# fractalclockwork/CS267_HW3

Hardware: NVIDIA B200
Metric: kmers_per_s_insert_plus_traverse (higher is better)
Workload: dtype u128

## Files before the change

### cs267_hw3_b200/csrc/capi.cu

```cuda
#include <algorithm>
#include <cmath>
#include <cstdio>
#include <cstdlib>
#include <cstring>
#include <string>
#include <vector>

#include <cub/device/device_radix_sort.cuh>

#include "../../include/kh_capi.h"
#include "kernels.cuh"
#include "ctable.cuh"

using namespace kh;

namespace {

struct DevBuf {
    void* p = nullptr;
    size_t cap = 0;
};

enum { EV_INS0, EV_INS1, EV_AS0, EV_WALK, EV_RANK, EV_AS1, EV_PACK0, EV_PACK1, EV_CLR0, EV_CLR1, EV_STAGE1, EV_BUILD0, EV_BUILD1, EV_COUNT };

// ... 33 lines not shown
    kh_stats stats = {};
    std::string err;
    int sm_count = 148, walk_blocks_per_sm = 0, rank_blocks_per_sm = 0;
    u64 last_contig_bytes = 0, last_n_contigs = 0;
    struct CtState {
        bool on = false, sealed = false, sharded = false, attr_set = false, connected = false;
        bool assembled = false;
        CtGeom g = {};
        CtCaps caps = {};
        CtPeers pe = {};
        u32 epoch = 0;
        u64 n_local_max = 0, n_total = 0, n_starts_max = 0, out_cap = 0;
        u64 n_starts_host = 0;
        DevBuf xin_vals, xin_chunk, xin_cnt, xin_done, xout_cursor, extra_vals, extra_chunk, extra_cnt, fine, chunk_cursor,
               chunk_base, pool_off, seg_base, ext_key, meta, pool, inbox, inbox_cnt, out_cursor, flags,
               answers, req_seg, g_link, g_meta, g_pool, g_hdr;
        bool slow = false;
        void* ipc_opened[kMaxRanks][24] = {};
    } ct;
    int ct_env = 1;
};

namespace {

int fail(kh_table* t, int status, const std::string& msg) {
    if (t) t->err = msg;
    return status;
}

#define KH_CUDA(t, expr)                                                                         \
    do {                                                                                         \
// ... 440 lines not shown
    KH_TRY(ensure(t, c.chunk_base, (C + 2) * sizeof(u32)));
    KH_TRY(ensure(t, c.pool_off, (C + 2) * sizeof(u32)));
    KH_TRY(ensure(t, c.seg_base, (C + 1) * sizeof(u32)));
    KH_TRY(ensure(t, c.pool, c.caps.pool_cap + 64));
    KH_TRY(ensure(t, c.inbox, (u64)world * c.caps.inbox_cap * sizeof(CtReq<W>)));
    KH_TRY(ensure(t, c.inbox_cnt, kMaxRanks * sizeof(u32)));
    KH_TRY(ensure(t, c.out_cursor, kMaxRanks * sizeof(u32)));
    KH_TRY(ensure(t, c.flags, 2 * kMaxRanks * sizeof(u32)));
    c.caps.g_seg_stride = world > 1 ? ((n_local_max + 1 + n_exp + 64 + 15) & ~15ull) : 0;
    c.caps.g_pool_stride = world > 1 ? ((c.caps.pool_cap + 64 + 15) & ~15ull) : 0;
    KH_TRY(ensure(t, c.answers, std::max<u64>(16, (u64)(world > 1 ? world : 0) * c.caps.inbox_cap * sizeof(u32))));
    KH_TRY(ensure(t, c.req_seg, std::max<u64>(16, (u64)(world > 1 ? world : 0) * c.caps.inbox_cap * sizeof(u32))));
    KH_TRY(ensure(t, c.g_link, std::max<u64>(16, (u64)world * c.caps.g_seg_stride * sizeof(u64))));
    KH_TRY(ensure(t, c.g_meta, std::max<u64>(16, (u64)world * c.caps.g_seg_stride * sizeof(u64))));
    KH_TRY(ensure(t, c.g_pool, std::max<u64>(16, (u64)world * c.caps.g_pool_stride)));
    KH_TRY(ensure(t, c.g_hdr, 2 * kMaxRanks * sizeof(u32)));
    if (sharded) {
        KH_TRY(ensure(t, t->link, seg_cap * sizeof(u64)));
        KH_TRY(ensure(t, c.meta, seg_cap * sizeof(u64)));
        KH_TRY(ensure(t, c.ext_key, seg_cap * sizeof(V)));
        KH_TRY(ensure(t, t->contig_len, (hcap + 2) * sizeof(u32)));
        KH_TRY(ensure(t, t->contig_pre, (hcap + 2) * sizeof(u32)));
        KH_TRY(ensure(t, t->contig_off, (hcap + 2) * sizeof(u64)));
        KH_TRY(ensure(t, t->out, c.out_cap));
        KH_TRY(ensure(t, t->starts, (hcap + 1) * sizeof(V)));
        const u64 ntiles = (n_local_max + kInsTile - 1) / kInsTile + 1;
        KH_TRY(ensure(t, t->mask, (ntiles + 1) * (kInsTile / 32) * sizeof(u32)));
        KH_TRY(ensure(t, t->tile_counts, (ntiles + 1) * sizeof(u32)));
        KH_TRY(ensure(t, t->tile_offs, (ntiles + 1) * sizeof(u64)));
        KH_TRY(ensure(t, t->scan_blocks, ((std::max(ntiles, hcap + 2) + kScanTile - 1) / kScanTile + 2) * sizeof(u64)));
    }
    KH_TRY(ct_reset_staging(t));
    KH_CUDA(t, cudaMemsetAsync(c.inbox_cnt.p, 0, kMaxRanks * sizeof(u32), t->stream));
    KH_CUDA(t, cudaMemsetAsync(c.flags.p, 0, 2 * kMaxRanks * sizeof(u32), t->stream));
// ... 83 lines not shown
    }
    return ct_barrier(t);
}
template <int W>
int ct_seal_build(kh_table* t) {
    typedef typename Slot<W>::value_t V;
    auto& c = t->ct;
    const u32 C = c.g.chunks_per_rank;
    if (!c.sharded) {
        const u64 hcap = c.n_starts_host + 1;
        const u64 seg_cap = hcap + std::max<u64>(t->n_expected, 1) + 64;
        if (seg_cap >= 0xFFFFFF00ull) return fail(t, KH_ERR_ARG, "too many segments for 32-bit ids");
        c.caps.hcap = (u32)hcap; c.caps.seg_cap = (u32)seg_cap;
        KH_TRY(ensure(t, t->link, seg_cap * sizeof(u64)));
        KH_TRY(ensure(t, c.meta, seg_cap * sizeof(u64)));
        KH_TRY(ensure(t, c.ext_key, seg_cap * sizeof(V)));
        ct_set_self(t);
    }
    ct_init_seal_kernel<<<1, 1, 0, t->stream>>>(t->d_ctr, c.caps.hcap);
    if (c.pe.world > 1) {
        u32* done = static_cast<u32*>(c.xin_done.p);
        ct_xin_scatter_kernel<W><<<(unsigned)t->sm_count * 8, 256, 0, t->stream>>>(
            static_cast<const V*>(c.xin_vals.p), static_cast<const u32*>(c.xin_chunk.p), static_cast<const u32*>(c.xin_cnt.p), done,
            c.g, c.caps, static_cast<u32*>(c.chunk_cursor.p), static_cast<V*>(c.fine.p), t->d_ctr);
        ct_extra_kernel<W><<<64, 256, 0, t->stream>>>(static_cast<const V*>(c.extra_vals.p), static_cast<const u32*>(c.extra_chunk.p),
                                                      static_cast<const u32*>(c.extra_cnt.p), done + kMaxRanks, c.caps, C,
                                                      static_cast<u32*>(c.chunk_cursor.p), static_cast<V*>(c.fine.p), t->d_ctr);
        ct_mark_filed_kernel<<<1, 32, 0, t->stream>>>(static_cast<const u32*>(c.xin_cnt.p), done, static_cast<const u32*>(c.extra_cnt.p),
                                                      done + kMaxRanks, c.caps, c.pe.world);
        t->n_launches += 3;
    }
    ct_layout_kernel<<<1, 1024, 0, t->stream>>>(static_cast<const u32*>(c.chunk_cursor.p), C, c.g, c.caps, (u32)Slot<W>::kPerBucket,
                                                CtBuild<W>::kMaxSlots, static_cast<u32*>(c.chunk_base.p), static_cast<u32*>(c.pool_off.p), t->d_ctr);
    t->n_launches += 2;
    KH_CUDA(t, cudaEventRecord(t->ev[EV_BUILD0], t->stream));
    ct_build_kernel<W><<<C, kCtBuildThreads, CtBuild<W>::kSmem, t->stream>>>(
        static_cast<const V*>(c.fine.p), static_cast<const u32*>(c.chunk_cursor.p), static_cast<const u32*>(c.chunk_base.p),
        static_cast<const u32*>(c.pool_off.p), static_cast<V*>(t->table), static_cast<u32*>(c.seg_base.p),
        static_cast<u64*>(t->link.p), static_cast<u64*>(c.meta.p), static_cast<V*>(c.ext_key.p),
        static_cast<unsigned char*>(c.pool.p), c.g, c.caps, t->d_ctr);
    KH_CUDA(t, cudaGetLastError());
    KH_CUDA(t, cudaEventRecord(t->ev[EV_BUILD1], t->stream));
    t->have_build = true;
    c.sealed = true;
    return KH_OK;
}

constexpr int kCtMaxRounds = 24;
constexpr int kCtParts = 8 + kCtMaxRounds;
constexpr u32 kCtWalkMaxSteps = 512;

template <int W>
int ct_assemble_part(kh_table* t, int part) {
    typedef typename Slot<W>::value_t V;
    auto& c = t->ct;
    const unsigned gb = (unsigned)t->sm_count * 8;
    u64* link = static_cast<u64*>(t->link.p);
    CtGathered gt = {};
    for (int r = 0; r < c.pe.world; ++r) {
        const bool me = r == c.pe.rank;
        gt.link[r] = me ? link : static_cast<const u64*>(c.g_link.p) + (u64)r * c.caps.g_seg_stride;
        gt.meta[r] = me ? static_cast<const u64*>(c.meta.p) : static_cast<const u64*>(c.g_meta.p) + (u64)r * c.caps.g_seg_stride;
        gt.pool[r] = me ? static_cast<const unsigned char*>(c.pool.p) : static_cast<const unsigned char*>(c.g_pool.p) + (u64)r * c.caps.g_pool_stride;
    }
    switch (part) {
    case 0:
        if (c.assembled) { c.sealed = false; c.assembled = false; }
        c.slow = false;
        KH_CUDA(t, cudaEventRecord(t->ev[EV_AS0], t->stream));
        if (!c.sealed) return ct_seal_publish<W>(t);
        return ct_barrier(t);
    case 1: {
        if (!c.sealed) { KH_TRY(ct_seal_build<W>(t)); KH_CUDA(t, cudaEventRecord(t->ev[EV_INS1], t->stream)); t->have_ins = true; }
        if (!c.sharded) {
            const u64 hc = c.n_starts_host;
            KH_TRY(ensure(t, t->contig_len, (hc + 3) * sizeof(u32)));
            KH_TRY(ensure(t, t->contig_pre, (hc + 3) * sizeof(u32)));
            KH_TRY(ensure(t, t->contig_off, (hc + 3) * sizeof(u64)));
// ... 30 lines not shown
        }
        return ct_barrier(t);
    case 3:
        if (c.pe.world > 1) {
            ct_apply_kernel<<<gb, 256, 0, t->stream>>>(link, static_cast<const u32*>(c.answers.p), static_cast<const u32*>(c.req_seg.p),
                                                       static_cast<const u32*>(c.out_cursor.p), c.caps, c.pe.world, c.pe.rank);
            ct_gather_kernel<<<gb, 256, 0, t->stream>>>(c.pe, c.caps, link, static_cast<const u64*>(c.meta.p), static_cast<const unsigned char*>(c.pool.p),
                                                        static_cast<const u32*>(c.pool_off.p), c.g.chunks_per_rank, t->d_ctr, 1);
            KH_CUDA(t, cudaStreamWaitEvent(t->stream, t->ev_gathered, 0));
            KH_CUDA(t, cudaGetLastError());
            t->n_launches += 2;
        }
        KH_CUDA(t, cudaEventRecord(t->ev[EV_WALK], t->stream));
        return ct_barrier(t);
    case 4:
        ct_walk_len_kernel<<<gb, 256, 0, t->stream>>>(gt, link, c.caps, t->k, kCtWalkMaxSteps, static_cast<u32*>(t->contig_len.p), t->d_ctr);
        KH_CUDA(t, cudaGetLastError());
        ++t->n_launches;
        return ct_barrier(t, -2);
    case 5: {
        KH_TRY(device_scan(t, static_cast<u32*>(t->contig_len.p), (u64)c.caps.hcap + 1, static_cast<u64*>(t->contig_off.p), &t->d_ctr->contig_bytes));
        KH_CUDA(t, cudaEventRecord(t->ev[EV_RANK], t->stream));
        ct_walk_emit_kernel<W><<<gb, 256, 0, t->stream>>>(gt, link, static_cast<const V*>(t->starts.p), c.caps, t->k, static_cast<const u32*>(t->contig_len.p),
                                                          static_cast<const u64*>(t->contig_off.p), c.out_cap, static_cast<char*>(t->out.p), t->d_ctr);
        KH_CUDA(t, cudaGetLastError());
        ++t->n_launches;
        KH_CUDA(t, cudaEventRecord(t->ev[EV_AS1], t->stream));
        t->have_as = true;
        return KH_OK;
    }
    case 6: {
        KH_TRY(read_counters(t));
        c.slow = (c.pe.world > 1 ? t->h_ctr->use_jump : t->h_ctr->need_jump) != 0;
        if (!c.slow) return KH_OK;
        c.assembled = true;
        ct_rank_round_kernel<<<gb, 256, 0, t->stream>>>(c.pe, link, c.caps, t->d_ctr, t->d_ctr->flags, 0);
        KH_CUDA(t, cudaGetLastError());
        ++t->n_launches;
        return ct_barrier(t, 0);
    }
    case 6 + kCtMaxRounds: {
        if (!c.slow) return KH_OK;
        ct_reset_nodes_kernel<<<1, 1, 0, t->stream>>>(t->d_ctr);
        ct_lengths_kernel<<<gb, 256, 0, t->stream>>>(c.pe, link, c.caps, t->k, static_cast<u32*>(t->contig_len.p),
                                                     static_cast<u32*>(t->contig_pre.p), t->d_ctr);
        ct_claim_kernel<<<gb, 256, 0, t->stream>>>(c.pe, link, c.caps, static_cast<const u32*>(t->contig_len.p), t->d_ctr);
        KH_CUDA(t, cudaGetLastError());
        t->n_launches += 3;
        KH_TRY(device_scan(t, static_cast<u32*>(t->contig_len.p), (u64)c.caps.hcap + 1, static_cast<u64*>(t->contig_off.p), &t->d_ctr->contig_bytes));
        KH_CUDA(t, cudaEventRecord(t->ev[EV_RANK], t->stream));
        return ct_barrier(t);
    }
    case 7 + kCtMaxRounds:
        if (!c.slow) return KH_OK;
        ct_emit_kernel<<<gb, 256, 0, t->stream>>>(c.pe, link, static_cast<const u64*>(c.meta.p), static_cast<const unsigned char*>(c.pool.p),
                                                  c.caps, t->d_ctr, t->k);
        ct_emit_heads_kernel<W><<<gb, 256, 0, t->stream>>>(static_cast<const V*>(t->starts.p), c.caps, t->k, static_cast<const u32*>(t->contig_len.p),
                                                          static_cast<const u64*>(t->contig_off.p), t->d_ctr, c.out_cap, static_cast<char*>(t->out.p));
        KH_CUDA(t, cudaGetLastError());
        t->n_launches += 2;
        KH_CUDA(t, cudaEventRecord(t->ev[EV_AS1], t->stream));
        t->have_as = true;
        return ct_barrier(t);
    default: {
        if (part < 7 || part >= 6 + kCtMaxRounds) return fail(t, KH_ERR_ARG, "unknown assemble part");
        if (!c.slow) return KH_OK;
        const int r = part - 6;
        ct_rank_round_kernel<<<gb, 256, 0, t->stream>>>(c.pe, link, c.caps, t->d_ctr, t->d_ctr->flags, r);
        KH_CUDA(t, cudaGetLastError());
        ++t->n_launches;
        return ct_barrier(t, r);
    }
    }
}

// ... 164 lines not shown
}

int kh_destroy(kh_table* t) {
    if (!t) return KH_OK;
    cudaSetDevice(t->device);
    if (t->own_stream) cudaStreamSynchronize(t->own_stream);
    DevBuf* bufs[] = {&t->starts, &t->mask, &t->tile_counts, &t->tile_offs, &t->scan_blocks, &t->link, &t->seglen,
                      &t->tmp, &t->part_cursor, &t->grouped, &t->fine, &t->chunk_cursor, &t->overflow, &t->contig_len, &t->contig_pre, &t->contig_off, &t->out, &t->stage[0], &t->stage[1],
                      &t->text_stage, &t->scratch_a, &t->scratch_b, &t->scratch_c, &t->sort_keys[0], &t->sort_keys[1], &t->sort_vals[0], &t->sort_vals[1], &t->sort_tmp};
    for (DevBuf* b : bufs) if (b->p) cudaFree(b->p);
    for (auto& row : t->ct.ipc_opened) for (void* q : row) if (q) cudaIpcCloseMemHandle(q);
    {
        auto& c = t->ct;
        for (DevBuf* b : {&c.xin_vals, &c.xin_chunk, &c.xin_cnt, &c.xin_done, &c.xout_cursor, &c.extra_vals, &c.extra_chunk, &c.extra_cnt, &c.fine,
                          &c.chunk_cursor, &c.chunk_base, &c.pool_off, &c.seg_base, &c.ext_key, &c.meta, &c.pool, &c.inbox, &c.inbox_cnt,
                          &c.out_cursor, &c.flags, &c.answers, &c.req_seg, &c.g_link, &c.g_meta, &c.g_pool, &c.g_hdr})
            if (b->p) cudaFree(b->p);
    }
    if (t->table) cudaFree(t->table);
    if (t->d_ctr) cudaFree(t->d_ctr);
    if (t->h_ctr) cudaFreeHost(t->h_ctr);
    if (t->h_out) cudaFreeHost(t->h_out);
    if (t->h_off) cudaFreeHost(t->h_off);
    for (auto& e : t->ev) if (e) cudaEventDestroy(e);
    for (auto& e : t->ev_copied) if (e) cudaEventDestroy(e);
    for (auto& e : t->ev_consumed) if (e) cudaEventDestroy(e);
    if (t->ev_built) cudaEventDestroy(t->ev_built);
    if (t->ev_gathered) cudaEventDestroy(t->ev_gathered);
    if (t->own_stream) cudaStreamDestroy(t->own_stream);
    if (t->copy_stream) cudaStreamDestroy(t->copy_stream);
    cudaGetLastError();
// ... 516 lines not shown
    if (offsets_dev) *offsets_dev = static_cast<const uint64_t*>(t->contig_off.p);
    if (n_contigs) *n_contigs = t->stats.n_contigs;
    if (contig_bytes) *contig_bytes = t->stats.contig_bytes;
    if (n_nodes) *n_nodes = t->stats.n_nodes;
    return KH_OK;
}

int kh_debug_buffer(kh_table* t, const char* name, void** ptr_out, uint64_t* bytes_out) {
    if (!t || !name || !ptr_out || !bytes_out) return KH_ERR_ARG;
    auto& c = t->ct;
    const std::string n(name);
    const DevBuf* b = nullptr;
    if (n == "link") b = &t->link; else if (n == "meta") b = &c.meta; else if (n == "ext_key") b = &c.ext_key;
    else if (n == "chunk_base") b = &c.chunk_base; else if (n == "seg_base") b = &c.seg_base; else if (n == "chunk_cursor") b = &c.chunk_cursor;
    else if (n == "inbox_cnt") b = &c.inbox_cnt; else if (n == "out_cursor") b = &c.out_cursor; else if (n == "xin_cnt") b = &c.xin_cnt;
    else if (n == "contig_len") b = &t->contig_len; else if (n == "pool") b = &c.pool;
    else if (n == "counters") { *ptr_out = t->d_ctr; *bytes_out = sizeof(Counters); return KH_OK; }
    else if (n == "caps") {
        static thread_local uint64_t v[8];
        v[0] = c.caps.hcap; v[1] = c.caps.seg_cap; v[2] = c.caps.inbox_cap; v[3] = c.caps.xin_cap; v[4] = c.g.chunks_per_rank; v[5] = 0;
        v[6] = c.epoch; v[7] = 0;
        *ptr_out = v; *bytes_out = sizeof(v); return KH_OK;
    }
    if (!b) return fail(t, KH_ERR_ARG, "unknown buffer " + n);
    *ptr_out = b->p; *bytes_out = b->cap;
    return KH_OK;
}

uint64_t kh_slot_bytes(int k) { return (ct_supported(k) ? ct_slot_words(k) : ((2 * k + 6 <= 64) ? 1 : 2)) * 8; }

int kh_copy_to_host(kh_table* t, void* dst_host, const void* src_dev, uint64_t bytes) {
// ... 29 lines not shown
```

### cs267_hw3_b200/csrc/ctable.cuh

```cuda
#pragma once
#include "kernels.cuh"

namespace kh {

#ifndef KH_CT_BUCKETS2
#define KH_CT_BUCKETS2 2176
#endif
#ifndef KH_CT_THREADS
#define KH_CT_THREADS 512
#endif
#ifndef KH_CT_MINBLOCKS
#define KH_CT_MINBLOCKS 2
#endif
#ifndef KH_CT_JUMPS
#define KH_CT_JUMPS 3
#endif
template <int W> struct CtBuild {
    static constexpr u32 kMaxBuckets = (W == 1) ? 1536u : (u32)KH_CT_BUCKETS2;
    static constexpr u32 kMaxSlots = kMaxBuckets * (u32)Slot<W>::kPerBucket;
    static constexpr u32 kOffSucc = kMaxBuckets * 32u;
    static constexpr u32 kOffPd = kOffSucc + kMaxSlots * 2u;
    static constexpr u32 kOffOff = kOffPd + kMaxSlots * 4u;
    static constexpr u32 kOffCode = kOffOff + kMaxSlots * 2u;
    static constexpr u32 kSmem = kOffCode + kMaxSlots;
};
constexpr int kCtBuildThreads = KH_CT_THREADS;
template <int W>
__host__ __device__ __forceinline__ u64 ct_fine_index(u32 chunk, u32 at, u32 nchunks) {
    constexpr u32 G = 128u / (u32)sizeof(typename Slot<W>::value_t);
    return ((u64)(at / G) * nchunks + chunk) * G + (at % G);
}
constexpr u32 kSuccExt = 0x8000u, kSuccTail = 0xFFFFu, kSuccDead = 0xFFFDu, kPredNone = 0xFFFFu;
constexpr u32 kCodeBackF = 8u, kCodeMulti = 16u;

template <int W> struct CtReq;
template <> struct alignas(16) CtReq<1> { u64 key; u32 src; u32 chunk; };
template <> struct alignas(16) CtReq<2> { u128 key; u32 src; u32 chunk; u64 pad; };

struct CtPeers {
    int world, rank;
    void* xin_vals[kMaxRanks];
    u32* xin_chunk[kMaxRanks];
    u32* xin_cnt[kMaxRanks];
    void* extra_vals[kMaxRanks];
    u32* extra_chunk[kMaxRanks];
    u32* extra_cnt[kMaxRanks];
    u64* link[kMaxRanks];
    u64* meta[kMaxRanks];
// ... 401 lines not shown
    int res = kFindNext;
#pragma unroll
    for (int i = 1; i >= 0; --i) {
        const bool e = ((u32)q[2 * i] & 7u) == 0u;
        const bool m = (((q[2 * i + 1] ^ key.hi) << kIdxBits) | ((q[2 * i] ^ key.lo) >> 6)) == 0ull;
        res = e ? kFindMiss : (m ? (int)(q[2 * i + 1] >> (64 - kIdxBits)) - 1 : res);
    }
    return res;
}

template <int W>
__global__ void __launch_bounds__(kCtBuildThreads, KH_CT_MINBLOCKS)
ct_build_kernel(const typename Slot<W>::value_t* __restrict__ fine, const u32* __restrict__ chunk_cursor,
                const u32* __restrict__ chunk_base, const u32* __restrict__ pool_off,
                typename Slot<W>::value_t* __restrict__ table, u32* __restrict__ seg_base,
                u64* __restrict__ link, u64* __restrict__ meta, typename Slot<W>::value_t* __restrict__ ext_key,
                unsigned char* __restrict__ pool, const CtGeom g, const CtCaps caps, Counters* ctr) {
    typedef Slot<W> S;
    typedef CtSlot<W> CS;
    typedef typename S::value_t V;
    typedef CtBuild<W> B;
    extern __shared__ __align__(128) unsigned char s_bld[];
    unsigned char* const s_raw = s_bld;
    V* s_tab = reinterpret_cast<V*>(s_raw);
    unsigned short* s_succ = reinterpret_cast<unsigned short*>(s_raw + B::kOffSucc);
    unsigned char* s_pool = s_raw + B::kOffSucc;
    u32* s_pd = reinterpret_cast<u32*>(s_raw + B::kOffPd);
    unsigned short* s_off = reinterpret_cast<unsigned short*>(s_raw + B::kOffOff);
    unsigned char* s_code = s_raw + B::kOffCode;
    __shared__ u32 s_inserted, s_dups, s_nheads, s_seg0, s_chars, s_err;
    const u32 c = blockIdx.x;
// ... 157 lines not shown
            if ((pa >> 16) != a) continue;
            const u32 f = s_code[node] & 7u;
            bool last = f == kExtF || s >= kSuccExt;
            u32 next_hi = f == kExtF ? kLinkTail : kLinkPending;
            if (!last) {
                const u32 ps = s_pd[s];
                if ((ps >> 16) == s) { last = true; next_hi = my_bits | (seg0 + (ps & 0xFFFFu)); }
            }
            if (!last) continue;
            const u32 n = (root ? 0u : (pd & 0xFFFFu)) + (f != kExtF ? 1u : 0u);
            const u32 off = atomicAdd(&s_chars, n);
            s_off[a] = (unsigned short)off;
            const u32 gseg = seg0 + (pa & 0xFFFFu);
            link[gseg] = ((u64)next_hi << 32) | (next_hi == kLinkTail ? 0u : n);
            meta[gseg] = ((pool0 + off) << 24) | n;
            if (next_hi == kLinkPending) ext_key[gseg] = S::next_key(CS::strip(s_tab[s & 0x7FFFu]), k);
        }
    }
    __syncthreads();
#pragma unroll 1
    for (u32 node = threadIdx.x; node < cnt; node += kCtBuildThreads) {
        const u32 code = s_code[node];
        if ((code & 7u) == kExtF) continue;
        const u32 pd = s_pd[node], a = pd >> 16;
        const bool root = a == node;
        if (!root && (s_pd[a] >> 16) != a) continue;
        s_pool[(u32)s_off[a] + (root ? 0u : (pd & 0xFFFFu))] = ext_char(code & 7u);
    }
    {
        const u32 nslots = nb * S::kPerBucket;
// ... 220 lines not shown
        if (what == 1) {
            for (u64 i = tid; i < cnt; i += stride) gl[first + i] = link[first + i];
        } else {
            for (u64 i = tid; i < cnt; i += stride) gm[first + i] = meta[first + i];
            const uint4* sp = reinterpret_cast<const uint4*>(pool);
            for (u64 i = tid; i < pool_vecs; i += stride) gp[i] = sp[i];
            if (tid == 0) { pe.g_hdr[p][2 * pe.rank] = nseg; pe.g_hdr[p][2 * pe.rank + 1] = (u32)pool_vecs; }
        }
    }
}

struct CtGathered {
    const u64* link[kMaxRanks];
    const u64* meta[kMaxRanks];
    const unsigned char* pool[kMaxRanks];
};

__global__ void __launch_bounds__(256)
ct_walk_len_kernel(const CtGathered gt, const u64* __restrict__ link, const CtCaps caps, int k, u32 max_steps,
                   u32* __restrict__ contig_len, Counters* ctr) {
    const u32 n_starts = (u32)min(ctr->n_starts_dev, (u64)caps.hcap);
    u64 nodes = 0;
    u32 err = 0, too_long = 0;
    for (u64 c = (u64)blockIdx.x * blockDim.x + threadIdx.x; c <= caps.hcap; c += (u64)gridDim.x * blockDim.x) {
        if (c >= n_starts) { contig_len[c] = 0; continue; }
        u32 gid = (u32)(__ldg(link + c) >> 32), chars = 0, e = 0, steps = 0;
        if (gid == kLinkMissing) e = kErrNotFound;
        else if (gid == kLinkConverge) e = kErrConverge;
        else if (gid >= kLinkCtFirstMarker) e = kErrInternal;
        while (!e) {
            const u64 l = __ldg(gt.link[gid >> kRankShift] + (gid & kLocalMask));
            const u32 hi = (u32)(l >> 32);
            if (hi == kLinkTail) { chars += (u32)(__ldg(gt.meta[gid >> kRankShift] + (gid & kLocalMask)) & 0xFFFFFFu); break; }
            if (hi == kLinkMissing) { e = kErrNotFound; break; }
            if (hi == kLinkConverge) { e = kErrConverge; break; }
            if (hi >= kLinkCtFirstMarker) { e = kErrInternal; break; }
            chars += (u32)l;
            gid = hi;
            if (++steps > max_steps) { too_long = 1; break; }
        }
        if (e || too_long) { err |= e; contig_len[c] = 0; continue; }
        contig_len[c] = (u32)k + chars + 1u;
        nodes += (u64)chars + 1u;
    }
    nodes = warp_sum_u64(nodes);
    err = __reduce_or_sync(kFullMask, err);
    too_long = __reduce_or_sync(kFullMask, too_long);
    if (lane_id() == 0) {
        if (nodes) atomicAdd(&ctr->n_nodes, nodes);
        if (err) atomicOr(&ctr->errors, err);
        if (err & kErrInternal) atomicOr(&ctr->err_where, kSiteStubOpen);
        if (too_long) atomicOr(&ctr->need_jump, 1u);
    }
}

__device__ __forceinline__ void ct_copy_chars(char* dst, const unsigned char* src, u32 n) {
    while (n && (reinterpret_cast<uintptr_t>(dst) & 3u)) { *dst++ = (char)*src++; --n; }
    if (n >= 4) {
        const u32 sh = ((u32)reinterpret_cast<uintptr_t>(src) & 3u) * 8u;
        const u32* sw = reinterpret_cast<const u32*>(reinterpret_cast<uintptr_t>(src) & ~(uintptr_t)3);
        u32 w0 = __ldg(sw);
        u32* dw = reinterpret_cast<u32*>(dst);
        const u32 nw = n >> 2;
        for (u32 i = 0; i < nw; ++i) {
            const u32 w1 = __ldg(sw + i + 1);
            dw[i] = __funnelshift_r(w0, w1, sh);
            w0 = w1;
        }
        dst += 4 * nw; src += 4 * nw; n &= 3u;
    }
    while (n) { *dst++ = (char)*src++; --n; }
}

template <int W>
__global__ void __launch_bounds__(256)
ct_walk_emit_kernel(const CtGathered gt, const u64* __restrict__ link, const typename Slot<W>::value_t* __restrict__ starts,
                    const CtCaps caps, int k, const u32* __restrict__ contig_len, const u64* __restrict__ contig_off, u64 out_cap,
                    char* __restrict__ out, const Counters* __restrict__ ctr) {
    typedef Slot<W> S;
    if (ctr->use_jump || ctr->need_jump || (ctr->errors & (kErrConverge | kErrCycle | kErrInternal | kErrNotFound)) || ctr->contig_bytes > out_cap) return;
    const u32 n_starts = (u32)min(ctr->n_starts_dev, (u64)caps.hcap);
    for (u64 c = (u64)blockIdx.x * blockDim.x + threadIdx.x; c < n_starts; c += (u64)gridDim.x * blockDim.x) {
        const u32 len = contig_len[c];
        if (len == 0) continue;
        char* dst = out + contig_off[c];
        char* const end = dst + len - 1u;
        *end = '\n';
        {
            const typename S::value_t v0 = starts[c];
            int j = 0;
            while (j < k && (reinterpret_cast<uintptr_t>(dst) & 3u)) { *dst++ = (char)ext_char(S::base_at(v0, k, j)); ++j; }
            for (; j + 4 <= k; j += 4, dst += 4) {
                const u32 w = (u32)ext_char(S::base_at(v0, k, j)) | ((u32)ext_char(S::base_at(v0, k, j + 1)) << 8) |
                              ((u32)ext_char(S::base_at(v0, k, j + 2)) << 16) | ((u32)ext_char(S::base_at(v0, k, j + 3)) << 24);
                *reinterpret_cast<u32*>(dst) = w;
            }
            for (; j < k; ++j) *dst++ = (char)ext_char(S::base_at(v0, k, j));
        }
        u32 gid = (u32)(__ldg(link + c) >> 32);
        for (;;) {
            const u32 r = gid >> kRankShift, i = gid & kLocalMask;
            const u64 l = __ldg(gt.link[r] + i), mt = __ldg(gt.meta[r] + i);
            const u32 n = (u32)(mt & 0xFFFFFFu);
            if (dst + n > end) break;
            ct_copy_chars(dst, gt.pool[r] + (mt >> 24), n);
            dst += n;
            const u32 hi = (u32)(l >> 32);
            if (hi >= kLinkCtFirstMarker) break;
            gid = hi;
        }
    }
}

__device__ __forceinline__ u64* ct_peer_link(const CtPeers& pe, u32 gid) { return pe.link[gid >> kRankShift] + (gid & kLocalMask); }
__device__ __forceinline__ bool ct_is_end_marker(u32 hi) { return hi == kLinkTail || hi == kLinkClaimed || hi == kLinkMissing || hi == kLinkConverge; }

__global__ void __launch_bounds__(256)
ct_rank_round_kernel(const CtPeers pe, u64* __restrict__ link, const CtCaps caps, Counters* ctr, u32* __restrict__ moved, int round) {
    if (ctr->rank_done || (round > 0 && moved[round - 1] == 0)) return;
    const u32 nseg = min(ctr->next_seg, caps.seg_cap);
    bool any = false;
    for (u64 i = (u64)blockIdx.x * blockDim.x + threadIdx.x; i < nseg; i += (u64)gridDim.x * blockDim.x) {
        const u64 li = __ldcg(link + i);
        const u32 pi = (u32)(li >> 32), si = (u32)li;
        if (pi >= kLinkCtFirstMarker) continue;
// ... 46 lines not shown
}

__global__ void __launch_bounds__(256)
ct_claim_kernel(const CtPeers pe, const u64* __restrict__ link, const CtCaps caps, const u32* __restrict__ contig_len, Counters* ctr) {
    const u32 n_starts = (u32)min(ctr->n_starts_dev, (u64)caps.hcap);
    for (u64 c = (u64)blockIdx.x * blockDim.x + threadIdx.x; c < n_starts; c += (u64)gridDim.x * blockDim.x) {
        if (contig_len[c] == 0) continue;
        const u32 tail = (u32)(__ldcg(link + c) >> 32);
        const u64 want = (u64)kLinkTail << 32;
        const u64 old = atomicCAS(ct_peer_link(pe, tail), want, ((u64)kLinkClaimed << 32) | (((u32)pe.rank << kRankShift) | (u32)c));
        if (old != want) atomicOr(&ctr->errors, kErrConverge);
    }
}

__global__ void __launch_bounds__(256)
ct_emit_kernel(const CtPeers pe, const u64* __restrict__ link, const u64* __restrict__ meta, const unsigned char* __restrict__ pool,
               const CtCaps caps, Counters* ctr, int k) {
    const u32 nseg = min(ctr->next_seg, caps.seg_cap);
    if (ctr->errors & (kErrConverge | kErrCycle | kErrInternal | kErrNotFound)) return;
    const u64 stride = (u64)gridDim.x * blockDim.x;
    for (u64 seg0 = (u64)caps.hcap + (u64)blockIdx.x * blockDim.x + (threadIdx.x & ~31u); seg0 < nseg; seg0 += stride) {
        const u64 seg = seg0 + lane_id();
        u32 len = 0;
        char* dst = nullptr;
        const unsigned char* src = nullptr;
        if (seg < nseg) {
            const u64 li = link[seg];
            const u32 pi = (u32)(li >> 32);
            const u64 mt = meta[seg];
            u32 cg = 0, dist = 0;
            bool ok = false, is_tail = false;
            if (pi == kLinkClaimed) { cg = (u32)li; ok = true; is_tail = true; }
            else if (pi < kLinkCtFirstMarker && ((u32)li & kLinkFinalBit)) {
                const u64 lt = *ct_peer_link(pe, pi);
                if ((u32)(lt >> 32) == kLinkClaimed) { cg = (u32)lt; dist = (u32)li & kLinkDistMask; ok = true; }
            }
            if (ok) {
                const u32 r = cg >> kRankShift, c = cg & kLocalMask;
                const u32 pre = pe.contig_pre[r][c];
                if (!is_tail && dist > pre) { atomicOr(&ctr->errors, kErrConverge); ok = false; }
                if (ok) {
                    const u64 off = pe.contig_off[r][c] + (u64)k + (is_tail ? pre : pre - dist);
                    len = (u32)(mt & 0xFFFFFFu);
                    if (off + len > pe.out_cap[r]) { ct_internal(ctr, kSiteOutCap); len = 0; }
                    dst = pe.out[r] + off;
                    src = pool + (mt >> 24);
                }
            }
        }
        u32 todo = __ballot_sync(kFullMask, len > 0);
        while (todo) {
            const int sl = __ffs(todo) - 1;
            todo &= todo - 1;
            const u32 n = __shfl_sync(kFullMask, len, sl);
            char* d = reinterpret_cast<char*>(__shfl_sync(kFullMask, reinterpret_cast<u64>(dst), sl));
            const unsigned char* s = reinterpret_cast<const unsigned char*>(__shfl_sync(kFullMask, reinterpret_cast<u64>(src), sl));
            for (u32 j = lane_id(); j < n; j += 32) d[j] = (char)s[j];
        }
    }
}

template <int W>
__global__ void __launch_bounds__(256)
ct_emit_heads_kernel(const typename Slot<W>::value_t* __restrict__ starts, const CtCaps caps, int k,
                     const u32* __restrict__ contig_len, const u64* __restrict__ contig_off,
                     const Counters* __restrict__ ctr, u64 out_cap, char* __restrict__ out) {
    typedef Slot<W> S;
    if (ctr->errors & (kErrConverge | kErrCycle | kErrInternal | kErrNotFound)) return;
    const u32 n_starts = (u32)min(ctr->n_starts_dev, (u64)caps.hcap);
    const u64 total = (u64)n_starts * (u32)(k + 1);
    for (u64 t = (u64)blockIdx.x * blockDim.x + threadIdx.x; t < total; t += (u64)gridDim.x * blockDim.x) {
        const u64 c = t / (u32)(k + 1);
        const u32 j = (u32)(t - c * (u32)(k + 1));
        const u32 len = contig_len[c];
        if (len == 0) continue;
        const u64 off = contig_off[c];
        if (off + len > out_cap) continue;
        if (j < (u32)k) out[off + j] = (char)ext_char(S::base_at(starts[c], k, (int)j));
        else out[off + len - 1] = '\n';
    }
}

template <int W>
__global__ void __launch_bounds__(256)
ct_scatter_starts_kernel(const unsigned char* __restrict__ recs, u64 n, int k, const u32* __restrict__ start_mask,
                         const u64* __restrict__ tile_offsets, u64 ntiles, typename Slot<W>::value_t* __restrict__ starts_out,
                         const Counters* __restrict__ ctr, u32 hcap) {
    typedef Slot<W> S;
    const u64 tile = ((u64)blockIdx.x * blockDim.x + threadIdx.x) >> 5;
    if (tile >= ntiles) return;
    const int pl = (k + 3) >> 2, pb = pl + 2;
    const u64 word = tile * (kInsTile / 32) + lane_id();
    const u64 nwords = (n + 31) >> 5;
    u32 m = word < nwords ? start_mask[word] : 0u;
// ... 23 lines not shown
```

Baseline: 12.65 billion.

## Replace per-contig serial emit walk with segment-parallel placement and warp-cooperative copy

The walk-length pass now records each segment's destination (contig id and offset) in a new seg_dst array. Output is then written by a segment-parallel kernel that uses a warp prefix sum and a balanced byte copy, and by a warp-cooperative kernel that writes the contig heads. This replaces the old emit kernel, in which one thread per contig chased links serially. The jumped path reuses the same emit after a placement kernel. The cost is an extra seg_dst buffer, an extra write per segment during the walk, and byte-granular stores in place of the old word-aligned copy.

```diff
diff --git a/cs267_hw3_b200/csrc/capi.cu b/cs267_hw3_b200/csrc/capi.cu
--- a/cs267_hw3_b200/csrc/capi.cu
+++ b/cs267_hw3_b200/csrc/capi.cu
@@ -71,7 +71,7 @@
         u64 n_starts_host = 0;
         DevBuf xin_vals, xin_chunk, xin_cnt, xin_done, xout_cursor, extra_vals, extra_chunk, extra_cnt, fine, chunk_cursor,
                chunk_base, pool_off, seg_base, ext_key, meta, pool, inbox, inbox_cnt, out_cursor, flags,
-               answers, req_seg, g_link, g_meta, g_pool, g_hdr;
+               answers, req_seg, g_link, g_meta, g_pool, g_hdr, seg_dst, g_seg_dst;
         bool slow = false;
         void* ipc_opened[kMaxRanks][24] = {};
     } ct;
@@ -542,10 +542,12 @@
     KH_TRY(ensure(t, c.g_link, std::max<u64>(16, (u64)world * c.caps.g_seg_stride * sizeof(u64))));
     KH_TRY(ensure(t, c.g_meta, std::max<u64>(16, (u64)world * c.caps.g_seg_stride * sizeof(u64))));
     KH_TRY(ensure(t, c.g_pool, std::max<u64>(16, (u64)world * c.caps.g_pool_stride)));
+    KH_TRY(ensure(t, c.g_seg_dst, std::max<u64>(16, (u64)world * c.caps.g_seg_stride * sizeof(u64))));
     KH_TRY(ensure(t, c.g_hdr, 2 * kMaxRanks * sizeof(u32)));
     if (sharded) {
         KH_TRY(ensure(t, t->link, seg_cap * sizeof(u64)));
         KH_TRY(ensure(t, c.meta, seg_cap * sizeof(u64)));
+        KH_TRY(ensure(t, c.seg_dst, seg_cap * sizeof(u64)));
         KH_TRY(ensure(t, c.ext_key, seg_cap * sizeof(V)));
         KH_TRY(ensure(t, t->contig_len, (hcap + 2) * sizeof(u32)));
         KH_TRY(ensure(t, t->contig_pre, (hcap + 2) * sizeof(u32)));
@@ -659,6 +661,7 @@
         c.caps.hcap = (u32)hcap; c.caps.seg_cap = (u32)seg_cap;
         KH_TRY(ensure(t, t->link, seg_cap * sizeof(u64)));
         KH_TRY(ensure(t, c.meta, seg_cap * sizeof(u64)));
+        KH_TRY(ensure(t, c.seg_dst, seg_cap * sizeof(u64)));
         KH_TRY(ensure(t, c.ext_key, seg_cap * sizeof(V)));
         ct_set_self(t);
     }
@@ -682,7 +685,7 @@
     ct_build_kernel<W><<<C, kCtBuildThreads, CtBuild<W>::kSmem, t->stream>>>(
         static_cast<const V*>(c.fine.p), static_cast<const u32*>(c.chunk_cursor.p), static_cast<const u32*>(c.chunk_base.p),
         static_cast<const u32*>(c.pool_off.p), static_cast<V*>(t->table), static_cast<u32*>(c.seg_base.p),
-        static_cast<u64*>(t->link.p), static_cast<u64*>(c.meta.p), static_cast<V*>(c.ext_key.p),
+        static_cast<u64*>(t->link.p), static_cast<u64*>(c.meta.p), static_cast<u64*>(c.seg_dst.p), static_cast<V*>(c.ext_key.p),
         static_cast<unsigned char*>(c.pool.p), c.g, c.caps, t->d_ctr);
     KH_CUDA(t, cudaGetLastError());
     KH_CUDA(t, cudaEventRecord(t->ev[EV_BUILD1], t->stream));
@@ -694,6 +697,19 @@
 constexpr int kCtMaxRounds = 24;
 constexpr int kCtParts = 8 + kCtMaxRounds;
 constexpr u32 kCtWalkMaxSteps = 512;
+
+template <int W>
+int ct_emit(kh_table* t, const CtGathered& gt, bool jumped) {
+    typedef typename Slot<W>::value_t V;
+    auto& c = t->ct;
+    const unsigned gb = (unsigned)t->sm_count * 8;
+    ct_emit_segments_kernel<<<gb, 256, 0, t->stream>>>(gt, c.pe, c.caps, t->k, jumped, t->d_ctr);
+    ct_emit_heads_kernel<W><<<gb, 256, 0, t->stream>>>(static_cast<const V*>(t->starts.p), c.caps, t->k, jumped, static_cast<const u32*>(t->contig_len.p),
+                                                      static_cast<const u64*>(t->contig_off.p), t->d_ctr, c.out_cap, static_cast<char*>(t->out.p));
+    KH_CUDA(t, cudaGetLastError());
+    t->n_launches += 2;
+    return KH_OK;
+}
 
 template <int W>
 int ct_assemble_part(kh_table* t, int part) {
@@ -707,6 +723,7 @@
         gt.link[r] = me ? link : static_cast<const u64*>(c.g_link.p) + (u64)r * c.caps.g_seg_stride;
         gt.meta[r] = me ? static_cast<const u64*>(c.meta.p) : static_cast<const u64*>(c.g_meta.p) + (u64)r * c.caps.g_seg_stride;
         gt.pool[r] = me ? static_cast<const unsigned char*>(c.pool.p) : static_cast<const unsigned char*>(c.g_pool.p) + (u64)r * c.caps.g_pool_stride;
+        gt.seg_dst[r] = me ? static_cast<u64*>(c.seg_dst.p) : static_cast<u64*>(c.g_seg_dst.p) + (u64)r * c.caps.g_seg_stride;
     }
     switch (part) {
     case 0:
@@ -767,17 +784,15 @@
         KH_CUDA(t, cudaEventRecord(t->ev[EV_WALK], t->stream));
         return ct_barrier(t);
     case 4:
-        ct_walk_len_kernel<<<gb, 256, 0, t->stream>>>(gt, link, c.caps, t->k, kCtWalkMaxSteps, static_cast<u32*>(t->contig_len.p), t->d_ctr);
+        if (c.pe.world > 1) { ct_unplace_gathered_kernel<<<gb, 256, 0, t->stream>>>(gt, c.pe, c.caps); ++t->n_launches; }
+        ct_walk_len_kernel<<<gb, 256, 0, t->stream>>>(gt, link, c.caps, t->k, c.pe.rank, kCtWalkMaxSteps, static_cast<u32*>(t->contig_len.p), t->d_ctr);
         KH_CUDA(t, cudaGetLastError());
         ++t->n_launches;
         return ct_barrier(t, -2);
     case 5: {
         KH_TRY(device_scan(t, static_cast<u32*>(t->contig_len.p), (u64)c.caps.hcap + 1, static_cast<u64*>(t->contig_off.p), &t->d_ctr->contig_bytes));
         KH_CUDA(t, cudaEventRecord(t->ev[EV_RANK], t->stream));
-        ct_walk_emit_kernel<W><<<gb, 256, 0, t->stream>>>(gt, link, static_cast<const V*>(t->starts.p), c.caps, t->k, static_cast<const u32*>(t->contig_len.p),
-                                                          static_cast<const u64*>(t->contig_off.p), c.out_cap, static_cast<char*>(t->out.p), t->d_ctr);
-        KH_CUDA(t, cudaGetLastError());
-        ++t->n_launches;
+        KH_TRY(ct_emit<W>(t, gt, false));
         KH_CUDA(t, cudaEventRecord(t->ev[EV_AS1], t->stream));
         t->have_as = true;
         return KH_OK;
@@ -806,12 +821,9 @@
     }
     case 7 + kCtMaxRounds:
         if (!c.slow) return KH_OK;
-        ct_emit_kernel<<<gb, 256, 0, t->stream>>>(c.pe, link, static_cast<const u64*>(c.meta.p), static_cast<const unsigned char*>(c.pool.p),
-                                                  c.caps, t->d_ctr, t->k);
-        ct_emit_heads_kernel<W><<<gb, 256, 0, t->stream>>>(static_cast<const V*>(t->starts.p), c.caps, t->k, static_cast<const u32*>(t->contig_len.p),
-                                                          static_cast<const u64*>(t->contig_off.p), t->d_ctr, c.out_cap, static_cast<char*>(t->out.p));
-        KH_CUDA(t, cudaGetLastError());
-        t->n_launches += 2;
+        ct_place_jumped_kernel<<<gb, 256, 0, t->stream>>>(c.pe, link, static_cast<u64*>(c.seg_dst.p), c.caps, t->d_ctr);
+        ++t->n_launches;
+        KH_TRY(ct_emit<W>(t, gt, true));
         KH_CUDA(t, cudaEventRecord(t->ev[EV_AS1], t->stream));
         t->have_as = true;
         return ct_barrier(t);
@@ -1006,7 +1018,7 @@
         auto& c = t->ct;
         for (DevBuf* b : {&c.xin_vals, &c.xin_chunk, &c.xin_cnt, &c.xin_done, &c.xout_cursor, &c.extra_vals, &c.extra_chunk, &c.extra_cnt, &c.fine,
                           &c.chunk_cursor, &c.chunk_base, &c.pool_off, &c.seg_base, &c.ext_key, &c.meta, &c.pool, &c.inbox, &c.inbox_cnt,
-                          &c.out_cursor, &c.flags, &c.answers, &c.req_seg, &c.g_link, &c.g_meta, &c.g_pool, &c.g_hdr})
+                          &c.out_cursor, &c.flags, &c.answers, &c.req_seg, &c.g_link, &c.g_meta, &c.g_pool, &c.g_hdr, &c.seg_dst, &c.g_seg_dst})
             if (b->p) cudaFree(b->p);
     }
     if (t->table) cudaFree(t->table);
@@ -1553,7 +1565,7 @@
     if (n == "link") b = &t->link; else if (n == "meta") b = &c.meta; else if (n == "ext_key") b = &c.ext_key;
     else if (n == "chunk_base") b = &c.chunk_base; else if (n == "seg_base") b = &c.seg_base; else if (n == "chunk_cursor") b = &c.chunk_cursor;
     else if (n == "inbox_cnt") b = &c.inbox_cnt; else if (n == "out_cursor") b = &c.out_cursor; else if (n == "xin_cnt") b = &c.xin_cnt;
-    else if (n == "contig_len") b = &t->contig_len; else if (n == "pool") b = &c.pool;
+    else if (n == "contig_len") b = &t->contig_len; else if (n == "pool") b = &c.pool; else if (n == "seg_dst") b = &c.seg_dst;
     else if (n == "counters") { *ptr_out = t->d_ctr; *bytes_out = sizeof(Counters); return KH_OK; }
     else if (n == "caps") {
         static thread_local uint64_t v[8];
diff --git a/cs267_hw3_b200/csrc/ctable.cuh b/cs267_hw3_b200/csrc/ctable.cuh
--- a/cs267_hw3_b200/csrc/ctable.cuh
+++ b/cs267_hw3_b200/csrc/ctable.cuh
@@ -32,6 +32,8 @@
 }
 constexpr u32 kSuccExt = 0x8000u, kSuccTail = 0xFFFFu, kSuccDead = 0xFFFDu, kPredNone = 0xFFFFu;
 constexpr u32 kCodeBackF = 8u, kCodeMulti = 16u;
+
+constexpr u64 kSegUnplaced = ~0ull;
 
 template <int W> struct CtReq;
 template <> struct alignas(16) CtReq<1> { u64 key; u32 src; u32 chunk; };
@@ -463,7 +465,7 @@
 ct_build_kernel(const typename Slot<W>::value_t* __restrict__ fine, const u32* __restrict__ chunk_cursor,
                 const u32* __restrict__ chunk_base, const u32* __restrict__ pool_off,
                 typename Slot<W>::value_t* __restrict__ table, u32* __restrict__ seg_base,
-                u64* __restrict__ link, u64* __restrict__ meta, typename Slot<W>::value_t* __restrict__ ext_key,
+                u64* __restrict__ link, u64* __restrict__ meta, u64* __restrict__ seg_dst, typename Slot<W>::value_t* __restrict__ ext_key,
                 unsigned char* __restrict__ pool, const CtGeom g, const CtCaps caps, Counters* ctr) {
     typedef Slot<W> S;
     typedef CtSlot<W> CS;
@@ -651,6 +653,7 @@
             const u32 gseg = seg0 + (pa & 0xFFFFu);
             link[gseg] = ((u64)next_hi << 32) | (next_hi == kLinkTail ? 0u : n);
             meta[gseg] = ((pool0 + off) << 24) | n;
+            seg_dst[gseg] = kSegUnplaced;
             if (next_hi == kLinkPending) ext_key[gseg] = S::next_key(CS::strip(s_tab[s & 0x7FFFu]), k);
         }
     }
@@ -901,12 +904,24 @@
     const u64* link[kMaxRanks];
     const u64* meta[kMaxRanks];
     const unsigned char* pool[kMaxRanks];
+    u64* seg_dst[kMaxRanks];
 };
 
 __global__ void __launch_bounds__(256)
-ct_walk_len_kernel(const CtGathered gt, const u64* __restrict__ link, const CtCaps caps, int k, u32 max_steps,
+ct_unplace_gathered_kernel(const CtGathered gt, const CtPeers pe, const CtCaps caps) {
+    const u64 tid = (u64)blockIdx.x * blockDim.x + threadIdx.x, stride = (u64)gridDim.x * blockDim.x;
+    for (int s = 0; s < pe.world; ++s) {
+        if (s == pe.rank) continue;
+        const u32 nseg = min(pe.g_hdr[pe.rank][2 * s], caps.seg_cap);
+        for (u64 i = caps.hcap + tid; i < nseg; i += stride) gt.seg_dst[s][i] = kSegUnplaced;
+    }
+}
+
+__global__ void __launch_bounds__(256)
+ct_walk_len_kernel(const CtGathered gt, const u64* __restrict__ link, const CtCaps caps, int k, int rank, u32 max_steps,
                    u32* __restrict__ contig_len, Counters* ctr) {
     const u32 n_starts = (u32)min(ctr->n_starts_dev, (u64)caps.hcap);
+    const u32 my_bits = (u32)rank << kRankShift;
     u64 nodes = 0;
     u32 err = 0, too_long = 0;
     for (u64 c = (u64)blockIdx.x * blockDim.x + threadIdx.x; c <= caps.hcap; c += (u64)gridDim.x * blockDim.x) {
@@ -915,13 +930,21 @@
         if (gid == kLinkMissing) e = kErrNotFound;
         else if (gid == kLinkConverge) e = kErrConverge;
         else if (gid >= kLinkCtFirstMarker) e = kErrInternal;
+        const u64 contig_bits = (u64)(my_bits | (u32)c) << 32;
         while (!e) {
-            const u64 l = __ldg(gt.link[gid >> kRankShift] + (gid & kLocalMask));
+            const u32 r = gid >> kRankShift, i = gid & kLocalMask;
+            const u64 l = __ldg(gt.link[r] + i);
             const u32 hi = (u32)(l >> 32);
-            if (hi == kLinkTail) { chars += (u32)(__ldg(gt.meta[gid >> kRankShift] + (gid & kLocalMask)) & 0xFFFFFFu); break; }
+            if (hi == kLinkTail) {
+                const u64 old = atomicCAS(reinterpret_cast<unsigned long long*>(gt.seg_dst[r] + i), kSegUnplaced, contig_bits | chars);
+                if (old != kSegUnplaced && old != (contig_bits | chars)) e = kErrConverge;
+                chars += (u32)(__ldg(gt.meta[r] + i) & 0xFFFFFFu);
+                break;
+            }
             if (hi == kLinkMissing) { e = kErrNotFound; break; }
             if (hi == kLinkConverge) { e = kErrConverge; break; }
             if (hi >= kLinkCtFirstMarker) { e = kErrInternal; break; }
+            gt.seg_dst[r][i] = contig_bits | chars;
             chars += (u32)l;
             gid = hi;
             if (++steps > max_steps) { too_long = 1; break; }
@@ -938,64 +961,6 @@
         if (err) atomicOr(&ctr->errors, err);
         if (err & kErrInternal) atomicOr(&ctr->err_where, kSiteStubOpen);
         if (too_long) atomicOr(&ctr->need_jump, 1u);
-    }
-}
-
-__device__ __forceinline__ void ct_copy_chars(char* dst, const unsigned char* src, u32 n) {
-    while (n && (reinterpret_cast<uintptr_t>(dst) & 3u)) { *dst++ = (char)*src++; --n; }
-    if (n >= 4) {
-        const u32 sh = ((u32)reinterpret_cast<uintptr_t>(src) & 3u) * 8u;
-        const u32* sw = reinterpret_cast<const u32*>(reinterpret_cast<uintptr_t>(src) & ~(uintptr_t)3);
-        u32 w0 = __ldg(sw);
-        u32* dw = reinterpret_cast<u32*>(dst);
-        const u32 nw = n >> 2;
-        for (u32 i = 0; i < nw; ++i) {
-            const u32 w1 = __ldg(sw + i + 1);
-            dw[i] = __funnelshift_r(w0, w1, sh);
-            w0 = w1;
-        }
-        dst += 4 * nw; src += 4 * nw; n &= 3u;
-    }
-    while (n) { *dst++ = (char)*src++; --n; }
-}
-
-template <int W>
-__global__ void __launch_bounds__(256)
-ct_walk_emit_kernel(const CtGathered gt, const u64* __restrict__ link, const typename Slot<W>::value_t* __restrict__ starts,
-                    const CtCaps caps, int k, const u32* __restrict__ contig_len, const u64* __restrict__ contig_off, u64 out_cap,
-                    char* __restrict__ out, const Counters* __restrict__ ctr) {
-    typedef Slot<W> S;
-    if (ctr->use_jump || ctr->need_jump || (ctr->errors & (kErrConverge | kErrCycle | kErrInternal | kErrNotFound)) || ctr->contig_bytes > out_cap) return;
-    const u32 n_starts = (u32)min(ctr->n_starts_dev, (u64)caps.hcap);
-    for (u64 c = (u64)blockIdx.x * blockDim.x + threadIdx.x; c < n_starts; c += (u64)gridDim.x * blockDim.x) {
-        const u32 len = contig_len[c];
-        if (len == 0) continue;
-        char* dst = out + contig_off[c];
-        char* const end = dst + len - 1u;
-        *end = '\n';
-        {
-            const typename S::value_t v0 = starts[c];
-            int j = 0;
-            while (j < k && (reinterpret_cast<uintptr_t>(dst) & 3u)) { *dst++ = (char)ext_char(S::base_at(v0, k, j)); ++j; }
-            for (; j + 4 <= k; j += 4, dst += 4) {
-                const u32 w = (u32)ext_char(S::base_at(v0, k, j)) | ((u32)ext_char(S::base_at(v0, k, j + 1)) << 8) |
-                              ((u32)ext_char(S::base_at(v0, k, j + 2)) << 16) | ((u32)ext_char(S::base_at(v0, k, j + 3)) << 24);
-                *reinterpret_cast<u32*>(dst) = w;
-            }
-            for (; j < k; ++j) *dst++ = (char)ext_char(S::base_at(v0, k, j));
-        }
-        u32 gid = (u32)(__ldg(link + c) >> 32);
-        for (;;) {
-            const u32 r = gid >> kRankShift, i = gid & kLocalMask;
-            const u64 l = __ldg(gt.link[r] + i), mt = __ldg(gt.meta[r] + i);
-            const u32 n = (u32)(mt & 0xFFFFFFu);
-            if (dst + n > end) break;
-            ct_copy_chars(dst, gt.pool[r] + (mt >> 24), n);
-            dst += n;
-            const u32 hi = (u32)(l >> 32);
-            if (hi >= kLinkCtFirstMarker) break;
-            gid = hi;
-        }
     }
 }
 
@@ -1072,70 +1037,118 @@
 }
 
 __global__ void __launch_bounds__(256)
-ct_emit_kernel(const CtPeers pe, const u64* __restrict__ link, const u64* __restrict__ meta, const unsigned char* __restrict__ pool,
-               const CtCaps caps, Counters* ctr, int k) {
+ct_place_jumped_kernel(const CtPeers pe, const u64* __restrict__ link, u64* __restrict__ seg_dst, const CtCaps caps, Counters* ctr) {
     const u32 nseg = min(ctr->next_seg, caps.seg_cap);
     if (ctr->errors & (kErrConverge | kErrCycle | kErrInternal | kErrNotFound)) return;
+    for (u64 seg = (u64)caps.hcap + (u64)blockIdx.x * blockDim.x + threadIdx.x; seg < nseg; seg += (u64)gridDim.x * blockDim.x) {
+        const u64 li = link[seg];
+        const u32 pi = (u32)(li >> 32);
+        u32 cg = 0, dist = 0;
+        bool ok = false, is_tail = false;
+        if (pi == kLinkClaimed) { cg = (u32)li; ok = true; is_tail = true; }
+        else if (pi < kLinkCtFirstMarker && ((u32)li & kLinkFinalBit)) {
+            const u64 lt = *ct_peer_link(pe, pi);
+            if ((u32)(lt >> 32) == kLinkClaimed) { cg = (u32)lt; dist = (u32)li & kLinkDistMask; ok = true; }
+        }
+        u64 place = kSegUnplaced;
+        if (ok) {
+            const u32 pre = pe.contig_pre[cg >> kRankShift][cg & kLocalMask];
+            if (!is_tail && dist > pre) atomicOr(&ctr->errors, kErrConverge);
+            else place = ((u64)cg << 32) | (is_tail ? pre : pre - dist);
+        }
+        seg_dst[seg] = place;
+    }
+}
+
+constexpr int kCopyUnroll = 4;
+__global__ void __launch_bounds__(256)
+ct_emit_segments_kernel(const CtGathered gt, const CtPeers pe, const CtCaps caps, int k, bool jumped, Counters* ctr) {
+    if ((!jumped && (ctr->use_jump || ctr->need_jump)) || (ctr->errors & (kErrConverge | kErrCycle | kErrInternal | kErrNotFound)) ||
+        ctr->contig_bytes > pe.out_cap[pe.rank]) return;
+    const bool multi = pe.world > 1;
     const u64 stride = (u64)gridDim.x * blockDim.x;
-    for (u64 seg0 = (u64)caps.hcap + (u64)blockIdx.x * blockDim.x + (threadIdx.x & ~31u); seg0 < nseg; seg0 += stride) {
-        const u64 seg = seg0 + lane_id();
-        u32 len = 0;
-        char* dst = nullptr;
-        const unsigned char* src = nullptr;
-        if (seg < nseg) {
-            const u64 li = link[seg];
-            const u32 pi = (u32)(li >> 32);
-            const u64 mt = meta[seg];
-            u32 cg = 0, dist = 0;
-            bool ok = false, is_tail = false;
-            if (pi == kLinkClaimed) { cg = (u32)li; ok = true; is_tail = true; }
-            else if (pi < kLinkCtFirstMarker && ((u32)li & kLinkFinalBit)) {
-                const u64 lt = *ct_peer_link(pe, pi);
-                if ((u32)(lt >> 32) == kLinkClaimed) { cg = (u32)lt; dist = (u32)li & kLinkDistMask; ok = true; }
-            }
-            if (ok) {
-                const u32 r = cg >> kRankShift, c = cg & kLocalMask;
-                const u32 pre = pe.contig_pre[r][c];
-                if (!is_tail && dist > pre) { atomicOr(&ctr->errors, kErrConverge); ok = false; }
-                if (ok) {
-                    const u64 off = pe.contig_off[r][c] + (u64)k + (is_tail ? pre : pre - dist);
+    const int nsrc = jumped ? 1 : pe.world;
+#pragma unroll 1
+    for (int i = 0; i < nsrc; ++i) {
+        const int s = jumped ? pe.rank : i;
+        const u32 nseg = s == pe.rank ? min(ctr->next_seg, caps.seg_cap) : min(pe.g_hdr[pe.rank][2 * s], caps.seg_cap);
+        const u64* __restrict__ meta = gt.meta[s];
+        const u64* __restrict__ seg_dst = gt.seg_dst[s];
+        const unsigned char* __restrict__ pool = gt.pool[s];
+        for (u64 seg0 = (u64)caps.hcap + (u64)blockIdx.x * blockDim.x + (threadIdx.x & ~31u); seg0 < nseg; seg0 += stride) {
+            const u64 seg = seg0 + lane_id();
+            u32 len = 0;
+            char* dst = nullptr;
+            const unsigned char* src = nullptr;
+            if (seg < nseg) {
+                const u64 sd = __ldcs(seg_dst + seg), mt = __ldcs(meta + seg);
+                if (sd != kSegUnplaced) {
+                    const u32 cg = (u32)(sd >> 32);
+                    const u32 r = multi ? cg >> kRankShift : 0u, c = multi ? cg & kLocalMask : cg;
+                    const u64 off = pe.contig_off[r][c] + (u64)k + (u32)sd;
                     len = (u32)(mt & 0xFFFFFFu);
                     if (off + len > pe.out_cap[r]) { ct_internal(ctr, kSiteOutCap); len = 0; }
                     dst = pe.out[r] + off;
                     src = pool + (mt >> 24);
                 }
             }
+            u32 incl = len;
+#pragma unroll
+            for (u32 d = 1; d < 32; d <<= 1) {
+                const u32 y = __shfl_up_sync(kFullMask, incl, d);
+                if (lane_id() >= d) incl += y;
+            }
+            const u32 excl = incl - len, total = __shfl_sync(kFullMask, incl, 31);
+            for (u32 base = 0; base < total; base += 32u * kCopyUnroll) {
+                unsigned char ch[kCopyUnroll];
+                char* to[kCopyUnroll];
+#pragma unroll
+                for (int q = 0; q < kCopyUnroll; ++q) {
+                    const u32 t = base + 32u * q + lane_id();
+                    u32 sl = 0;
+#pragma unroll
+                    for (u32 step = 16; step; step >>= 1)
+                        if (__shfl_sync(kFullMask, excl, sl + step) <= t) sl += step;
+                    const u32 o = t - __shfl_sync(kFullMask, excl, sl);
+                    const unsigned char* p = reinterpret_cast<const unsigned char*>(__shfl_sync(kFullMask, reinterpret_cast<u64>(src), sl));
+                    char* d = reinterpret_cast<char*>(__shfl_sync(kFullMask, reinterpret_cast<u64>(dst), sl));
+                    to[q] = t < total ? d + o : nullptr;
+                    ch[q] = t < total ? __ldcs(p + o) : (unsigned char)0;
+                }
+#pragma unroll
+                for (int q = 0; q < kCopyUnroll; ++q)
+                    if (to[q]) *to[q] = (char)ch[q];
+            }
+        }
+    }
+}
+
+template <int W>
+__global__ void __launch_bounds__(256)
+ct_emit_heads_kernel(const typename Slot<W>::value_t* __restrict__ starts, const CtCaps caps, int k, bool jumped,
+                     const u32* __restrict__ contig_len, const u64* __restrict__ contig_off,
+                     const Counters* __restrict__ ctr, u64 out_cap, char* __restrict__ out) {
+    typedef Slot<W> S;
+    if ((!jumped && (ctr->use_jump || ctr->need_jump)) || (ctr->errors & (kErrConverge | kErrCycle | kErrInternal | kErrNotFound)) ||
+        ctr->contig_bytes > out_cap) return;
+    const u32 n_starts = (u32)min(ctr->n_starts_dev, (u64)caps.hcap);
+    const u64 stride = (u64)gridDim.x * blockDim.x;
+    for (u64 c0 = (u64)blockIdx.x * blockDim.x + (threadIdx.x & ~31u); c0 < n_starts; c0 += stride) {
+        const u64 c = c0 + lane_id();
+        u32 len = 0;
+        char* dst = nullptr;
+        if (c < n_starts) {
+            len = contig_len[c];
+            if (len) { dst = out + contig_off[c]; dst[len - 1u] = '\n'; }
         }
         u32 todo = __ballot_sync(kFullMask, len > 0);
         while (todo) {
             const int sl = __ffs(todo) - 1;
             todo &= todo - 1;
-            const u32 n = __shfl_sync(kFullMask, len, sl);
             char* d = reinterpret_cast<char*>(__shfl_sync(kFullMask, reinterpret_cast<u64>(dst), sl));
-            const unsigned char* s = reinterpret_cast<const unsigned char*>(__shfl_sync(kFullMask, reinterpret_cast<u64>(src), sl));
-            for (u32 j = lane_id(); j < n; j += 32) d[j] = (char)s[j];
-        }
-    }
-}
-
-template <int W>
-__global__ void __launch_bounds__(256)
-ct_emit_heads_kernel(const typename Slot<W>::value_t* __restrict__ starts, const CtCaps caps, int k,
-                     const u32* __restrict__ contig_len, const u64* __restrict__ contig_off,
-                     const Counters* __restrict__ ctr, u64 out_cap, char* __restrict__ out) {
-    typedef Slot<W> S;
-    if (ctr->errors & (kErrConverge | kErrCycle | kErrInternal | kErrNotFound)) return;
-    const u32 n_starts = (u32)min(ctr->n_starts_dev, (u64)caps.hcap);
-    const u64 total = (u64)n_starts * (u32)(k + 1);
-    for (u64 t = (u64)blockIdx.x * blockDim.x + threadIdx.x; t < total; t += (u64)gridDim.x * blockDim.x) {
-        const u64 c = t / (u32)(k + 1);
-        const u32 j = (u32)(t - c * (u32)(k + 1));
-        const u32 len = contig_len[c];
-        if (len == 0) continue;
-        const u64 off = contig_off[c];
-        if (off + len > out_cap) continue;
-        if (j < (u32)k) out[off + j] = (char)ext_char(S::base_at(starts[c], k, (int)j));
-        else out[off + len - 1] = '\n';
+            const typename S::value_t v0 = starts[c0 + sl];
+            for (int j = (int)lane_id(); j < k; j += 32) d[j] = (char)ext_char(S::base_at(v0, k, j));
+        }
     }
 }
 
```

Measured after the change: 12.80 billion (median of 6 runs). 1.2% higher.
